# dusk-network/dusk-blindbidproof

Measured on AMD Instinct MI355X. Metric: blind-bid proofs/sec, higher is better.
Workload: dtype u32

## Files before the change

### __graft_entry__.py

```python
import os
import shutil
import subprocess
import sys

ROOT = os.path.dirname(os.path.abspath(__file__))
PKG = os.path.join(ROOT, "dusk_blindbidproof_amd")
CSRC = os.path.join(PKG, "csrc")
LIB = os.path.join(PKG, "libbbp_hip.so")
ORACLE_SO = os.path.join(ROOT, "oracle", "_build", "libbbp_oracle.so")
HOSTCHECK_SO = os.path.join(ROOT, "tests", "_build", "libhostcheck.so")
DEVCHECK_SO = {"chain": os.path.join(ROOT, "tests", "_build", "libbbp_devcheck.so"),
               "nochain": os.path.join(ROOT, "tests", "_build", "libbbp_devcheck_nochain.so")}
DEVCHECK_DEFS = {"chain": [], "nochain": ["-DBBP_FE_NO_CHAIN"]}


def _newer(target, sources):
    if not os.path.exists(target):
        return True
    t = os.path.getmtime(target)
    return any(os.path.getmtime(s) > t for s in sources)


def _run(cmd):
    print("+", " ".join(cmd), flush=True)
# ... 138 lines not shown
        _run(["g++", "-O1", "-g", "-std=c++17", "-fsanitize=address,undefined", "-fno-sanitize-recover=all", "-o", WIRE_FUZZ_BIN, src])
    return WIRE_FUZZ_BIN


VERIFY_PLAN_SAN_BIN = os.path.join(ROOT, "tests", "_build", "verify_plan_san")


def build_verify_plan_san(force=False):
    src = os.path.join(ROOT, "tests", "verify_plan_san.cpp")
    if force or _newer(VERIFY_PLAN_SAN_BIN, [src, os.path.join(ROOT, "tests", "host_check.cpp")] + _csrc_files((".h", ".inc"))):
        os.makedirs(os.path.dirname(VERIFY_PLAN_SAN_BIN), exist_ok=True)
        _run(["g++", "-O1", "-g", "-std=c++17", "-fsanitize=address,undefined", "-fno-sanitize-recover=all", "-o", VERIFY_PLAN_SAN_BIN, src])
    return VERIFY_PLAN_SAN_BIN


COMBINER_TSAN_BIN = os.path.join(ROOT, "tests", "_build", "combiner_tsan")


def build_combiner_tsan(force=False):
    srcs = [os.path.join(ROOT, "tests", "combiner_tsan.cpp"), os.path.join(CSRC, "submit.cpp")]
    if force or _newer(COMBINER_TSAN_BIN, srcs + [os.path.join(CSRC, "submit.h")]):
        os.makedirs(os.path.dirname(COMBINER_TSAN_BIN), exist_ok=True)
        _run(["g++", "-O1", "-g", "-std=c++17", "-fsanitize=thread", "-pthread", "-o", COMBINER_TSAN_BIN] + srcs)
    return COMBINER_TSAN_BIN


COMBINER_RULES_BIN = os.path.join(ROOT, "tests", "_build", "combiner_rules")


def build_combiner_rules(force=False):
# ... 56 lines not shown
```

### dusk_blindbidproof_amd/csrc/context.h

```cpp
#pragma once
#include <hip/hip_runtime.h>
#include <stdint.h>
#include <stdio.h>
#include <stdlib.h>
#include <string.h>

#include <atomic>
#include <condition_variable>
#include <map>
#include <mutex>
#include <new>
#include <stdexcept>
#include <string>
#include <vector>

#include "../../include/bbp.h"
#include "point.h"
#include "msm_plan.h"
#include "prove_io.h"
#include "prove_plan.h"
#include "scalar.h"
#include "verify_plan.h"
#include "verify_rows.h"

namespace bbp {

constexpr int MSM_POS = 256;
#ifndef BBP_MSM_T
#define BBP_MSM_T 128
#endif
constexpr int MSM_T = BBP_MSM_T;
#ifndef BBP_ACC_T
#define BBP_ACC_T 256
#endif
constexpr int ACC_T = BBP_ACC_T;
static_assert(ACC_T % MSM_T == 0, "the fold kernel deals the accumulate kernel's chunks to its lanes");
constexpr int MSM_G = MSM_K / MSM_T;
constexpr int MSM_LOG_G = MSM_T == 128 ? 3 : 4;
static_assert(MSM_T == 128 || MSM_T == 64, "the cross-lane fold is written for one or two wavefronts");
constexpr int FOLD_CLS = 2048 >> (FOLD_ROUND - 1);
constexpr int FOLD_NAF = 9;
constexpr int FOLD_W = 29;
constexpr int FOLD_M = 128;
constexpr int FOLD_K = FOLD_CLS * FOLD_M;
static_assert(SMALL_W == FOLD_W, "split MSMs recode at the generator-fold pass's width");
constexpr int PAD_BASES = 202;
constexpr unsigned PAD_BASE0 = BBP_NUM_BASES;
constexpr unsigned MRG_BASE0 = PAD_BASE0 + PAD_BASES;
constexpr int MRG_BASES = 2 * 2048;
constexpr unsigned MSM_SKIP_BASE = 0xffffffffu;
constexpr unsigned TAB_BASES = BBP_NUM_BASES + PAD_BASES + MRG_BASES;
constexpr int GE_WORDS = sizeof(ge) / 4;

struct DevBuf {
    void* p = nullptr;
    size_t cap = 0;
};

}

// ... 10 lines not shown
    hipStream_t copy = nullptr;
    hipStream_t side2 = nullptr;
    bbp::ProveKnobs knobs;
    bbp::ProveRuleState prove_state;
    bbp::VerifyKnobs vknobs;
    std::vector<hipStream_t> spare_streams;
    static constexpr int CALL_RING = 8;
    hipEvent_t ev_call[CALL_RING] = {};
    bool ev_call_valid[CALL_RING] = {};
    int last_prove_par = -1;
    static constexpr int MAX_SLICES = bbp::PROVE_MAX_SLICES;
    hipStream_t lane[MAX_SLICES] = {nullptr, nullptr, nullptr, nullptr};
    hipEvent_t ev_join[MAX_SLICES] = {nullptr, nullptr, nullptr, nullptr}, ev_stagger[MAX_SLICES] = {nullptr, nullptr, nullptr, nullptr};
    bbp::MsmKnobs msm_knobs;
    bool sort_lds_attr = false;
    bool sort_lds_attr1 = false;
    int debug_corrupt = 0;
    std::map<const void*, int> serial_attr;
    static constexpr int PROVE_BUFS = bbp::PROVE_BUFS;
    hipEvent_t ev_open[PROVE_BUFS] = {}, ev_done[PROVE_BUFS] = {};
    hipEvent_t ev_entry[PROVE_BUFS] = {};
    bool ev_done_valid[PROVE_BUFS] = {}, ev_open_valid[PROVE_BUFS] = {};
    int verify_serial_acc = 0;
    static constexpr int VACC_RING = 4;
    hipEvent_t ev_vacc[VACC_RING] = {};
    uint32_t vacc_seq = 0;
    bool vacc_valid = false;
    uint32_t seq_at_last_verify = 0;
    hipEvent_t ev_prep = nullptr;
    bool ev_prep_valid = false;
    hipEvent_t ev_draw = nullptr;
// ... 245 lines not shown
int hw_queues_state();
int32_t pool_prove_batch(bbp_ctx* pool, uint32_t B, uint32_t N, const uint8_t* in, const uint8_t* entropy, uint8_t* out, int32_t* status);
int32_t pool_prove_round(bbp_ctx* pool, uint32_t N, const uint8_t* round, uint32_t B, const uint8_t* bids, const uint8_t* entropy, uint8_t* rows_out,
                         uint64_t* toggles_out, int32_t* status);
int32_t pool_verify(bbp_ctx* pool, const VerifyRows& rows, const uint8_t* in, int32_t* status, uint32_t group, uint32_t* n_fallback);
int32_t verify_host(bbp_ctx* ctx, const VerifyRows& rows, const uint8_t* in, int32_t* status, uint32_t group, uint32_t* n_fallback);
int32_t pool_msm_batch(bbp_ctx* pool, uint32_t B, uint32_t n_terms, const uint8_t* scalars, uint32_t layout, uint8_t* out32);
int32_t pool_reject(bbp_ctx* pool, const char* what);
void pool_workers_start(bbp_ctx* pool);
void pool_workers_stop(bbp_ctx* pool);
int pool_member_numa_node(const bbp_ctx* pool, uint32_t i);

int32_t msm_launch(bbp_ctx* ctx, uint32_t n_msm, uint32_t n_terms, const u32* scalars_dev, const u32* base_idx_dev,
                   ge* out_points_dev, hipStream_t stream, uint32_t n_idx_sets = 1, int scratch_slot = 0, const u32* msm_map_dev = nullptr,
                   const u32* n_active_dev = nullptr, bool chain_acc = false);
int32_t fold_generators_launch(bbp_ctx* ctx, uint32_t n_proofs, const sc* g_dev, const sc* h_dev, ge* out_dev, hipStream_t stream,
                               int scratch_slot);
int32_t encode_launch(bbp_ctx* ctx, uint32_t n, const ge* pts_dev, uint8_t* out32_dev, hipStream_t stream);
size_t msm_scratch_bytes(uint32_t n_msm, uint32_t n_terms);
int32_t tail_btab_build(bbp_ctx* ctx);
size_t tail_btab_bytes();

}
```

### dusk_blindbidproof_amd/csrc/msm.hip

```cpp
#include "context.h"

namespace bbp {

#ifndef BBP_FOLD_PRIO
#define BBP_FOLD_PRIO 2
#endif
#ifndef BBP_MSM_WAVES
#define BBP_MSM_WAVES 2
#endif
#ifndef BBP_MSM_WAVES_MAX
#define BBP_MSM_WAVES_MAX 2
#endif

#ifdef BBP_MSM_PROF
__device__ unsigned long long g_msm_prof[8];
#define MSM_PROF_BEGIN() unsigned long long prof_t = wall_clock64()
#define MSM_PROF_MARK(i)                                                    \
    if (tid == 0) {                                                         \
        unsigned long long now_ = wall_clock64();                           \
        atomicAdd(&g_msm_prof[i], now_ - prof_t);                           \
        prof_t = now_;                                                      \
    }
#else
#define MSM_PROF_BEGIN()
// ... 87 lines not shown

template <int MODE>
__global__ __launch_bounds__(SORT_T) void k_msm_sort(const u32* __restrict__ scal_a, const u32* __restrict__ aux, u32 n_total, u32 n_idx_sets,
                                                      u32 n_sub, u32 split, u32* __restrict__ sorted_all, u32* __restrict__ cursor_all,
                                                      const u32* __restrict__ msm_map, const u32* __restrict__ n_active, u32* __restrict__ ticket) {
    constexpr int K = msm_geom<MODE>::K, NAF = msm_geom<MODE>::NAF, W = msm_geom<MODE>::W, G = K >= SORT_T ? K / SORT_T : 1;
    __shared__ u32 cursor[K + 1];
    __shared__ u32 part[SORT_T];
    const int tid = threadIdx.x;
    if (ticket && blockIdx.x == 0 && tid == 0) *ticket = 0;
    if (n_active && blockIdx.x >= *n_active) return;
    const size_t work = blockIdx.x, msm = work / split;
    const u32 i0 = (u32)(work % split) * n_sub;
    const u32 n = i0 < n_total ? min(n_sub, n_total - i0) : 0u;
    __builtin_amdgcn_s_setprio(3);
    const u32* sbase;
    const u32* base_idx = nullptr;
    u32 base0 = 0;
    if (MODE != 1) {
        const size_t src = msm_map ? (size_t)msm_map[msm] : msm;
        sbase = scal_a + (src * (size_t)n_total + i0) * 8;
        base_idx = aux + (size_t)(msm % n_idx_sets) * n_total + i0;
    } else {
        const u32 side = (u32)msm & 1u;
        sbase = (side ? aux : scal_a) + ((msm >> 1) * (size_t)2048 + i0) * 8;
        base0 = (side ? BBP_BASE_H0 : BBP_BASE_G0) + i0;
    }
    u32* sorted = sorted_all + work * (size_t)n_sub * W;
    auto key = [&](u32 i, u32 mag) -> u32 { return (MODE != 1 ? 0u : ((i0 + i) & (FOLD_CLS - 1)) * FOLD_M) + ((mag + 1) >> 1); };

    for (int k = tid; k <= K; k += SORT_T) cursor[k] = 0;
    __syncthreads();
    for (u32 i = tid; i < n; i += SORT_T) {
        const uint4* sp = reinterpret_cast<const uint4*>(sbase + (size_t)i * 8);
        uint4 lo = sp[0], hi = sp[1];
        const u32 s[8] = {lo.x, lo.y, lo.z, lo.w, hi.x, hi.y, hi.z, hi.w};
        if (MODE != 1 && base_idx[i] == MSM_SKIP_BASE) continue;
        sc_for_each_naf_digit<NAF>(s, [&](u32, u32 mag, u32) { atomicAdd(&cursor[key(i, mag)], 1u); });
    }
    __syncthreads();
    {
        u32 local = 0;
        for (int r = 1; r <= G; r++)
            if (tid * G + r <= K) local += cursor[tid * G + r];
        const int lane = tid & 63, wave = tid >> 6;
        u32 incl = local;
#pragma unroll
        for (int d = 1; d < 64; d <<= 1) {
            const u32 up = (u32)__shfl_up((int)incl, d, 64);
            if (lane >= d) incl += up;
        }
        if (lane == 63) part[wave] = incl;
// ... 10 lines not shown
        }
        __syncthreads();
        u32 base = part[wave] + incl - local;
        for (int r = 1; r <= G; r++) {
            if (tid * G + r > K) break;
            const u32 c = cursor[tid * G + r];
            cursor[tid * G + r] = base;
            base += c;
        }
    }
    __syncthreads();
    for (u32 i = tid; i < n; i += SORT_T) {
        const uint4* sp = reinterpret_cast<const uint4*>(sbase + (size_t)i * 8);
        uint4 lo = sp[0], hi = sp[1];
        const u32 s[8] = {lo.x, lo.y, lo.z, lo.w, hi.x, hi.y, hi.z, hi.w};
        if (MODE != 1 && base_idx[i] == MSM_SKIP_BASE) continue;
        const u32 tb = (MODE != 1 ? base_idx[i] : base0 + i) * MSM_POS;
        sc_for_each_naf_digit<NAF>(s, [&](u32 pos, u32 mag, u32 neg) {
            u32 at = atomicAdd(&cursor[key(i, mag)], 1u);
            sorted[at] = (tb + pos) | (neg << 31);
        });
    }
    __syncthreads();
    u32* cur_out = cursor_all + work * (size_t)(K + 1);
    for (int k = tid; k <= K; k += SORT_T) cur_out[k] = k ? cursor[k] : 0u;
}

template <int MODE> struct sort_cap { static constexpr u32 V = BBP_SORT_CAP; };
template <> struct sort_cap<1> { static constexpr u32 V = 8192; };

template <int MODE>
__global__ __launch_bounds__(SORT_T) void k_msm_sort_staged(const u32* __restrict__ scal_a, const u32* __restrict__ aux, u32 n_total, u32 n_idx_sets,
                                                             u32 n_sub, u32 split, u32* __restrict__ sorted_all, u32* __restrict__ cursor_all,
                                                             const u32* __restrict__ msm_map, const u32* __restrict__ n_active, u32 CAP, u32* __restrict__ ticket) {
    constexpr int K = msm_geom<MODE>::K, NAF = msm_geom<MODE>::NAF, W = msm_geom<MODE>::W, G = K >= SORT_T ? K / SORT_T : 1;
    extern __shared__ u32 stage[];
    __shared__ u32 start[K + 2];
    __shared__ u32 fill[K + 1];
    __shared__ u32 part[SORT_T];
    const int tid = threadIdx.x;
    if (ticket && blockIdx.x == 0 && tid == 0) *ticket = 0;
    if (n_active && blockIdx.x >= *n_active) return;
    const size_t work = blockIdx.x, msm = work / split;
    const u32 i0 = (u32)(work % split) * n_sub;
    const u32 n = i0 < n_total ? min(n_sub, n_total - i0) : 0u;
    __builtin_amdgcn_s_setprio(3);
    const u32* sbase;
    const u32* base_idx = nullptr;
    u32 base0 = 0;
    if (MODE != 1) {
        const size_t src = msm_map ? (size_t)msm_map[msm] : msm;
        sbase = scal_a + (src * (size_t)n_total + i0) * 8;
        base_idx = aux + (size_t)(msm % n_idx_sets) * n_total + i0;
    } else {
        const u32 side = (u32)msm & 1u;
        sbase = (side ? aux : scal_a) + ((msm >> 1) * (size_t)2048 + i0) * 8;
        base0 = (side ? BBP_BASE_H0 : BBP_BASE_G0) + i0;
    }
    u32* sorted = sorted_all + work * (size_t)n_sub * W;
    auto key = [&](u32 i, u32 mag) -> u32 { return (MODE != 1 ? 0u : ((i0 + i) & (FOLD_CLS - 1)) * FOLD_M) + ((mag + 1) >> 1); };

    for (int k = tid; k <= K; k += SORT_T) fill[k] = 0;
    __syncthreads();
    for (u32 i = tid; i < n; i += SORT_T) {
        const uint4* sp = reinterpret_cast<const uint4*>(sbase + (size_t)i * 8);
        uint4 lo = sp[0], hi = sp[1];
        const u32 s[8] = {lo.x, lo.y, lo.z, lo.w, hi.x, hi.y, hi.z, hi.w};
        if (MODE != 1 && base_idx[i] == MSM_SKIP_BASE) continue;
        sc_for_each_naf_digit<NAF>(s, [&](u32, u32 mag, u32) { atomicAdd(&fill[key(i, mag)], 1u); });
    }
    __syncthreads();
    {
        u32 local = 0;
        for (int r = 1; r <= G; r++)
            if (tid * G + r <= K) local += fill[tid * G + r];
        const int lane = tid & 63, wave = tid >> 6;
        u32 incl = local;
#pragma unroll
        for (int d = 1; d < 64; d <<= 1) {
            const u32 up = (u32)__shfl_up((int)incl, d, 64);
            if (lane >= d) incl += up;
        }
        if (lane == 63) part[wave] = incl;
// ... 27 lines not shown
        const bool direct = start[kb + 1] - base > CAP;
        u32 ke = kb + 1;
        if (!direct) {
            u32 lo = kb + 1, hi = (u32)K + 1;
            while (lo < hi) {
                const u32 mid = (lo + hi + 1) >> 1;
                if (start[mid] - base <= CAP) lo = mid; else hi = mid - 1;
            }
            ke = lo;
        }
        if (start[ke] != base) {
            for (u32 i = tid; i < n; i += SORT_T) {
                const uint4* sp = reinterpret_cast<const uint4*>(sbase + (size_t)i * 8);
                uint4 lo4 = sp[0], hi4 = sp[1];
                const u32 s[8] = {lo4.x, lo4.y, lo4.z, lo4.w, hi4.x, hi4.y, hi4.z, hi4.w};
                if (MODE != 1 && base_idx[i] == MSM_SKIP_BASE) continue;
                const u32 tb = (MODE != 1 ? base_idx[i] : base0 + i) * MSM_POS;
                sc_for_each_naf_digit<NAF>(s, [&](u32 pos, u32 mag, u32 neg) {
                    const u32 k = key(i, mag);
                    if (k >= kb && k < ke) {
                        const u32 at = start[k] + atomicAdd(&fill[k], 1u);
                        const u32 ent = (tb + pos) | (neg << 31);
                        if (direct) sorted[at] = ent; else stage[at - base] = ent;
                    }
                });
            }
            __syncthreads();
            if (!direct) {
                const u32 cnt = start[ke] - base;
                for (u32 i = tid; i < cnt; i += SORT_T) sorted[base + i] = stage[i];
            }
            __syncthreads();
        }
        kb = ke;
    }
    u32* cur_out = cursor_all + work * (size_t)(K + 1);
    for (int k = tid; k <= K; k += SORT_T) cur_out[k] = k ? start[k + 1] : 0u;
}

#ifndef BBP_ACC_WG
#define BBP_ACC_WG 256
#endif
constexpr int ACC_WG = BBP_ACC_WG, ACC_WGS = ACC_T / ACC_WG;
static_assert(ACC_T % ACC_WG == 0 && ACC_WG % 64 == 0, "accumulate workgroup geometry");

template <int MODE>
__global__ __launch_bounds__(ACC_WG) __attribute__((amdgpu_waves_per_eu(BBP_MSM_WAVES, BBP_MSM_WAVES_MAX)))
void k_msm_acc(const niels_row* __restrict__ ptable, const u32* __restrict__ sorted_all, const u32* __restrict__ cursor_all, u32 n ,
               ge* __restrict__ bsum_all, ge* __restrict__ psum_all, ge* __restrict__ out, const u32* __restrict__ n_active, u32* __restrict__ fault,
               u32 n_work, u32* __restrict__ ticket) {
    constexpr int K = msm_geom<MODE>::K, W = msm_geom<MODE>::W, G = K / MSM_T;
    __shared__ u32 cursor[K + 1];
// ... 113 lines not shown
        *dest = acc;
    }
#endif
#ifdef BBP_MSM_PROF
    if (tid == 0) atomicAdd(&g_msm_prof[6], clock64() - clk0);
#endif
    MSM_PROF_MARK(2);
    __threadfence_block();
    __syncthreads();
    MSM_PROF_MARK(3);
#ifdef BBP_ACC_PERSIST
  }
#endif
}

template <int MODE>
__global__ __launch_bounds__(MSM_T) void k_msm_fold(const u32* __restrict__ cursor_all, ge* __restrict__ bsum_all, const ge* __restrict__ psum_all,
                                                     ge* __restrict__ out, const u32* __restrict__ n_active) {
    constexpr int K = msm_geom<MODE>::K, G = K / MSM_T;
    __shared__ u32 cursor[K + 1];
    __shared__ u32 xch[GE_WORDS];
    const int tid = threadIdx.x;
    if (n_active && blockIdx.x >= *n_active) return;
    __builtin_amdgcn_s_setprio(BBP_FOLD_PRIO);
    const size_t msm = blockIdx.x;
    {
        const u32* cur_in = cursor_all + msm * (size_t)(K + 1);
        for (int k = tid; k <= K; k += MSM_T) cursor[k] = cur_in[k];
    }
    __syncthreads();
    const u32 E = cursor[K];
    ge* bsum = bsum_all + msm * (size_t)K;
    const ge* psum = psum_all + msm * (size_t)ACC_T;
#ifdef BBP_KO_FOLD
    if (MODE != 1) { if (tid == 0) out[msm] = bsum[0]; }
    else if (tid < FOLD_CLS) out[msm * FOLD_CLS + tid] = bsum[tid];
    return;
#endif
    for (u32 ch = tid; ch < (u32)ACC_T; ch += MSM_T) {
        const u32 c0 = (u32)(((u64)ch * E) / ACC_T), c1 = (u32)(((u64)(ch + 1) * E) / ACC_T);
        if (c0 >= c1) continue;
        u32 lo = 1, hi = K;
        while (lo < hi) {
            u32 mid = (lo + hi) >> 1;
            if (cursor[mid] > c0) hi = mid; else lo = mid + 1;
        }
        const u32 k_first = lo;
        const bool inside = cursor[lo - 1] < c0;
        const bool last_of_run = inside && !(c1 < E && c1 > cursor[k_first - 1] && c1 < cursor[k_first]);
        if (last_of_run) {
            ge part = psum[ch];
            for (int u = (int)ch - 1; u >= 0; u--) {
                const u32 cu = (u32)(((u64)u * E) / ACC_T), cu1 = (u32)(((u64)(u + 1) * E) / ACC_T);
                if (cu <= cursor[k_first - 1]) break;
                if (cu1 > cu) ge_add_nc(part, part, psum[u]);
            }
            ge head = bsum[k_first - 1];
            ge_add_nc(head, head, part);
            bsum[k_first - 1] = head;
        }
    }
    __threadfence_block();
    __syncthreads();

    ge running = ge_identity(), total = ge_identity();
    if constexpr (G == 1) {
        if (cursor[tid + 1] != cursor[tid]) running = bsum[tid];
        total = running;
    } else {
#pragma unroll 1
        for (int r = G; r >= 1; r--) {
            const u32 k = tid * G + r;
            if (cursor[k] != cursor[k - 1]) running = ge_add(running, bsum[k - 1]);
            total = ge_add(total, running);
        }
    }

    if constexpr (MODE != 1) {
        const int lane = tid & 63, wave = tid >> 6;
#pragma unroll 1
        for (int d = 1; d < 64; d <<= 1) {
            ge other = ge_shfl_down(running, d);
            if (lane + d < 64) running = ge_add(running, other);
        }
        if (MSM_T > 64) {
            if (tid == 64) xch_put(xch, running);
            __syncthreads();
            if (wave == 0) {
// ... 228 lines not shown
#pragma unroll 1
    for (int d = REDUCE_L / 2; d >= 1; d >>= 1) {
        const ge other = ge_shfl_down(acc, d);
        if ((int)j < d) acc = ge_add(acc, other);
    }
    if (o < n_out && j == 0) out[o] = acc;
}


struct MsmScratch {
    u32 *sorted, *cursor;
    ge *bsum, *psum, *tmp;
    u32* ticket;
    size_t bytes;
};
static MsmScratch msm_scratch_layout(void* base, size_t n_msm, size_t n_terms, size_t W, size_t K, size_t out_items = 1) {
    auto up = [](size_t x) { return (x + 255) / 256 * 256; };
    MsmScratch m;
    size_t o = 0;
    m.sorted = reinterpret_cast<u32*>(static_cast<u8*>(base) + o);
    o += up(n_msm * n_terms * W * sizeof(u32));
    m.cursor = reinterpret_cast<u32*>(static_cast<u8*>(base) + o);
    o += up(n_msm * (K + 1) * sizeof(u32));
    m.bsum = reinterpret_cast<ge*>(static_cast<u8*>(base) + o);
    o += n_msm * K * sizeof(ge);
    m.psum = reinterpret_cast<ge*>(static_cast<u8*>(base) + o);
    o += n_msm * ACC_T * sizeof(ge);
    m.tmp = reinterpret_cast<ge*>(static_cast<u8*>(base) + o);
    o += up(n_msm * out_items * sizeof(ge));
    m.ticket = reinterpret_cast<u32*>(static_cast<u8*>(base) + o);
    o += 256;
    m.bytes = o;
    return m;
}
size_t msm_scratch_bytes(uint32_t n_msm, uint32_t n_terms) {
    const u32 split = msm_split(n_msm, n_terms), n_sub = (n_terms + split - 1) / split;
    size_t a = msm_scratch_layout(nullptr, (size_t)n_msm * split, n_sub, MSM_W, MSM_K).bytes;
    if (split > 1) a = std::max(a, msm_scratch_layout(nullptr, (size_t)n_msm * split, n_sub, SMALL_W, SMALL_K).bytes);
    const size_t b = msm_scratch_layout(nullptr, n_msm, n_terms, MSM_W, MSM_K).bytes;
    return a > b ? a : b;
}

static inline u32 acc_grid(bbp_ctx*, u32 n_work) {
#ifdef BBP_ACC_PERSIST
    static const u32 cap = [] { const char* e = getenv("BBP_ACC_PERSIST_GRID"); return e ? (u32)atoi(e) : 512u; }();
    return n_work < cap ? n_work : cap;
#else
    return n_work * ACC_WGS;
#endif
}

int32_t fold_generators_launch(bbp_ctx* ctx, uint32_t n_proofs, const sc* g_dev, const sc* h_dev, ge* out_dev, hipStream_t stream,
                               int scratch_slot) {
    if (n_proofs == 0) return BBP_OK;
    const size_t n_msm = 2 * (size_t)n_proofs;
    const u32 split = msm_split((u32)n_msm, 2048), n_sub = (2048 + split - 1) / split;
    const size_t n_work = n_msm * split;
    DevBuf& scratch = ctx->slice_fold[scratch_slot];
    int32_t rc = dev_reserve(ctx, scratch, msm_scratch_layout(nullptr, n_work, n_sub, FOLD_W, FOLD_K, FOLD_CLS).bytes);
    if (rc) return rc;
    const MsmScratch m = msm_scratch_layout(scratch.p, n_work, n_sub, FOLD_W, FOLD_K, FOLD_CLS);
    {
        ScopedEvent ev(ctx, TAG_MSM_SORT, stream);
        if (ctx->msm_knobs.sort_staged & 2) {
            if (!ctx->sort_lds_attr1) {
                BBP_HIP_TRY(ctx, hipFuncSetAttribute((const void*)k_msm_sort_staged<1>, hipFuncAttributeMaxDynamicSharedMemorySize, (int)(sort_cap<1>::V * 4)));
                ctx->sort_lds_attr1 = true;
            }
            hipLaunchKernelGGL(k_msm_sort_staged<1>, dim3((u32)n_work), dim3(SORT_T), sort_cap<1>::V * 4, stream, (const u32*)g_dev, (const u32*)h_dev, 2048u, 1u,
                               n_sub, split, m.sorted, m.cursor, (const u32*)nullptr, (const u32*)nullptr, sort_cap<1>::V, m.ticket);
        } else
            hipLaunchKernelGGL(k_msm_sort<1>, dim3((u32)n_work), dim3(SORT_T), 0, stream, (const u32*)g_dev, (const u32*)h_dev, 2048u, 1u, n_sub, split,
                               m.sorted, m.cursor, (const u32*)nullptr, (const u32*)nullptr, m.ticket);
        BBP_HIP_TRY(ctx, hipGetLastError());
    }
    {
        ScopedEvent ev(ctx, TAG_MSM, stream);
        hipLaunchKernelGGL(k_msm_acc<1>, dim3(acc_grid(ctx, (u32)n_work)), dim3(ACC_WG), 0, stream, ctx->ptable, m.sorted, m.cursor, n_sub, m.bsum, m.psum,
                           split > 1 ? m.tmp : out_dev, (const u32*)nullptr, ctx->health, (u32)n_work, m.ticket);
        BBP_HIP_TRY(ctx, hipGetLastError());
    }
    ScopedEvent evf(ctx, TAG_MSM_FOLD, stream);
    hipLaunchKernelGGL(k_msm_fold<1>, dim3((u32)n_work), dim3(MSM_T), 0, stream, m.cursor, m.bsum, m.psum, split > 1 ? m.tmp : out_dev,
                       (const u32*)nullptr);
    BBP_HIP_TRY(ctx, hipGetLastError());
    if (split > 1) {
        const u32 n_out = (u32)n_msm * FOLD_CLS;
        hipLaunchKernelGGL(k_msm_reduce, dim3((n_out * REDUCE_L + 63) / 64), dim3(64), lds_token(ctx), stream, n_out, split, (u32)FOLD_CLS, m.tmp, out_dev);
        BBP_HIP_TRY(ctx, hipGetLastError());
    }
    return BBP_OK;
}

__global__ __launch_bounds__(64) void k_encode(const ge* __restrict__ pts, u32 n, u32* __restrict__ out_words) {
    u32 i = blockIdx.x * blockDim.x + threadIdx.x;
    if (i >= n) return;
    ge p = pts[i];
    u32 w[8];
    ge_encode_words(w, p);
    uint4* o = reinterpret_cast<uint4*>(out_words + (size_t)i * 8);
    o[0] = make_uint4(w[0], w[1], w[2], w[3]);
    o[1] = make_uint4(w[4], w[5], w[6], w[7]);
}
// ... 120 lines not shown
```

### dusk_blindbidproof_amd/csrc/msm_plan.h

```cpp
#pragma once
#include <stdint.h>
#include <stdlib.h>
#include <string.h>

#include <initializer_list>

namespace bbp {

constexpr int MSM_NAF = 12;
constexpr int MSM_W = 22;
constexpr int MSM_K = 1 << (MSM_NAF - 2);
constexpr int SMALL_NAF = 9;
constexpr int SMALL_K = 1 << (SMALL_NAF - 2);
constexpr int SMALL_W = 29;

#ifndef BBP_SORT_CAP
#define BBP_SORT_CAP 21504
#endif
constexpr uint32_t SORT_CAP_WIDE = 32768;
constexpr uint32_t SORT_WIDE_FROM = 3000;
constexpr uint32_t MSM_SPLIT_MAX = 16;

struct MsmKnobs {
    int sort_staged = 3;
// ... 64 lines not shown
    p.reduce = p.split > 1;
    if (p.split > 1 && k.msm_small) {
        p.geom = MsmPlan::SMALL;
        p.fold = MsmPlan::SMALL_FOLD;
        return p;
    }
    const bool wide = p.n_sub > SORT_WIDE_FROM;
    if ((k.sort_staged & 1) && (!wide || (k.sort_staged & 4))) {
        p.sort = wide ? MsmPlan::STAGED_WIDE : MsmPlan::STAGED;
        p.sort_cap = wide ? SORT_CAP_WIDE : (uint32_t)BBP_SORT_CAP;
    }
    p.fold = p.n_work >= (uint32_t)k.fold_half_from ? MsmPlan::HALF : MsmPlan::LANES128;
    return p;
}

}
```

### dusk_blindbidproof_amd/csrc/prover.hip

```cpp
#define BBP_KECCAK_WAVE 1
#include <string.h>

#include <functional>

#include "batch.h"
#include "hosthash.h"
#include "keccak_wave.h"
#include "scalarmul.h"
#include "witness.h"

namespace bbp {

#define BBP_THIN_PRIO() __builtin_amdgcn_s_setprio(3)
#ifndef BBP_LANE_KERNEL
#define BBP_LANE_KERNEL __launch_bounds__(64)
#endif


__device__ __forceinline__ void sc_to_bytes32(uint8_t* o, const sc& s) { sc_tobytes(o, s); }
__device__ __forceinline__ void words_to_bytes32(uint8_t* o, const u32* w) {
#pragma unroll
    for (int i = 0; i < 8; i++) {
        o[4 * i] = (uint8_t)w[i];
        o[4 * i + 1] = (uint8_t)(w[i] >> 8);
// ... 858 lines not shown
    for (int k = 0; k < TAIL_PIECES; k++) {
        ge cur = P;
        T[8 * k] = P;
#pragma unroll 1
        for (int i = 1; i < 8; i++) {
            cur = ge_add(cur, P);
            T[8 * k + i] = cur;
        }
        if (k < TAIL_PIECES - 1) {
#pragma unroll 1
            for (int i = 0; i < TAIL_PIECE_BITS; i++) P = ge_dbl(P);
        }
    }
}

__global__ void k_tail_init(u32 B, sc* __restrict__ g_all, sc* __restrict__ h_all) {
    BBP_THIN_PRIO();
    u32 t = blockIdx.x * blockDim.x + threadIdx.x;
    if (t >= B * FOLD_CLS) return;
    const u32 p = t / FOLD_CLS, k = t % FOLD_CLS;
    st_sc(&g_all[(size_t)p * 2048 + k], sc_one());
    st_sc(&h_all[(size_t)p * 2048 + k], sc_one());
}

#ifndef BBP_TAIL_SPLIT
#define BBP_TAIL_SPLIT 1
#endif
#ifndef BBP_TAIL_MERGE
#define BBP_TAIL_MERGE 1
#endif
#ifndef BBP_TAIL_BLK
#define BBP_TAIL_BLK (BBP_TAIL_SPLIT == 1 ? 256 : 320)
#endif
constexpr int TAIL_SPLIT = BBP_TAIL_SPLIT, TAIL_MERGE = BBP_TAIL_MERGE, TAIL_LS = TAIL_MERGE == 2 ? 17 : 33 * TAIL_SPLIT, TAIL_BLK = BBP_TAIL_BLK, TAIL_LP = 2 * TAIL_LS, TAIL_PPB = TAIL_BLK / TAIL_LP;
static_assert(TAIL_PIECES % TAIL_SPLIT == 0 && TAIL_PPB >= 1 && (TAIL_MERGE == 1 || (TAIL_MERGE == 2 && TAIL_SPLIT == 1)), "tail kernel geometry");
__global__ __launch_bounds__(TAIL_BLK) void k_tail_lr(u32 B, u32 n, u32 prev_round, u32 m, const u32* __restrict__ enc, merlin_transcript* __restrict__ tr,
                                                       const sc* __restrict__ misc, sc* __restrict__ a_all, sc* __restrict__ b_all,
// ... 485 lines not shown
    for (u32 r = 1; r <= 11 && r < tail_from; r++) {
        if (r > 1) LAUNCH(ctx, TAG_TRANSCRIPT, k_ipa_challenge, tgrid, 64, s, B, r - 1, m, bd.enc, bd.tr, bd.misc, tw);
        if (hp.wide_ipa)
            LAUNCH(ctx, TAG_IPA_SCALARS, k_ipa_round<IPA_BLK_WIDE>, B, IPA_BLK_WIDE, s, r, n1, bd.misc, bd.a, bd.b, bd.g, bd.h, bd.lr);
        else
            LAUNCH(ctx, TAG_IPA_SCALARS, k_ipa_round<IPA_BLK>, B, IPA_BLK, s, r, n1, bd.misc, bd.a, bd.b, bd.g, bd.h, bd.lr);
        if ((rc = msm_launch(ctx, 2 * B, 2049, (const u32*)bd.lr, c.idx_ipa + (size_t)(r - 1) * 2 * 2049, bd.lrpts, s, 2, slot))) return rc;
        LAUNCH(ctx, TAG_ENCODE, k_encode_strided, cdiv(2 * B, 64), 64, s, 2 * B, 2u, bd.lrpts, 2u, bd.enc, encw, 8 * (m + 8 + 2 * (r - 1)), 1u);
    }
    if (tail_from <= 11) {
        DevBuf& vt = ctx->slice_vtab[slot];
        if ((rc = dev_reserve(ctx, vt, (size_t)B * 2 * FOLD_CLS * TAIL_TAB * sizeof(ge)))) return rc;
        ge* ftab = static_cast<ge*>(vt.p);
        LAUNCH(ctx, TAG_TRANSCRIPT, k_ipa_challenge, tgrid, 64, s, B, tail_from - 1, m, bd.enc, bd.tr, bd.misc, tw);
        LAUNCH(ctx, TAG_IPA_SCALARS, k_ipa_round<IPA_BLK>, B, IPA_BLK, s, tail_from, n1, bd.misc, bd.a, bd.b, bd.g, bd.h, (sc*)nullptr);
        if ((rc = fold_generators_launch(ctx, B, bd.g, bd.h, bd.fpts, s, slot))) return rc;
        LAUNCH(ctx, TAG_VARBASE, k_tail_init, cdiv(B * FOLD_CLS, 64), 64, s, B, bd.g, bd.h);
        LAUNCH(ctx, TAG_VARBASE, k_tail_tables, cdiv(B * 2 * FOLD_CLS, 64), 64, s, B * 2 * FOLD_CLS, bd.fpts, ftab);
        for (u32 r = tail_from; r <= 11; r++) {
            const u32 n = 1024u >> (r - 1);
            LAUNCH(ctx, TAG_VARBASE, k_tail_lr, cdiv(B, TAIL_PPB), TAIL_BLK, s, B, n, r > tail_from ? r - 1 : 0u, m, bd.enc, bd.tr, bd.misc, bd.a, bd.b, bd.g, bd.h, ftab,
                   ctx->btab, bd.lrpts);
            LAUNCH(ctx, TAG_ENCODE, k_encode_strided, cdiv(2 * B, 64), 64, s, 2 * B, 2u, bd.lrpts, 2u, bd.enc, encw, 8 * (m + 8 + 2 * (r - 1)), 1u);
        }
    }
    LAUNCH(ctx, TAG_TRANSCRIPT, k_ipa_final, tgrid, 64, s, B, m, bd.enc, bd.tr, bd.misc, bd.a, bd.b, tw);
    if (out_guard) BBP_HIP_TRY(ctx, hipStreamWaitEvent(s, out_guard, 0));
    LAUNCH(ctx, TAG_TRANSCRIPT, k_assemble, cdiv(B, 64), 64, s, B, m, bd.enc, bd.misc, out_dev);
    return BBP_OK;
}

int32_t debug_read_misc(bbp_ctx* ctx, u32 B, u32 N, u32 proof, uint8_t* out) {
// ... 13 lines not shown
```

Baseline: 22650.

## Replace generator-fold MSM with dedicated class-strided fold sort and accumulate kernels

Swaps the generic MODE-1 MSM sort/accumulate path for folding generators with new k_fold_sort and k_fold_acc kernels. The sort bins one scalar per class stride into 128 buckets, and each accumulate lane handles one class, so the per-class bucket key expansion goes away. The fold now takes n1 and the u challenge so it can handle the partially-active boundary generator. k_tail_init seeds h with yipow instead of one, which shifts the y-inverse factor out of the folded scalars. A new FoldPlan computes the scratch layout. Correctness depends on the tag and class masking logic being exact.

```diff
diff --git a/__graft_entry__.py b/__graft_entry__.py
--- a/__graft_entry__.py
+++ b/__graft_entry__.py
@@ -176,6 +176,17 @@
     return VERIFY_PLAN_SAN_BIN
 
 
+FOLD_PLAN_SAN_BIN = os.path.join(ROOT, "tests", "_build", "fold_plan_san")
+
+
+def build_fold_plan_san(force=False):
+    src = os.path.join(ROOT, "tests", "fold_plan_san.cpp")
+    if force or _newer(FOLD_PLAN_SAN_BIN, [src, os.path.join(CSRC, "msm_plan.h")]):
+        os.makedirs(os.path.dirname(FOLD_PLAN_SAN_BIN), exist_ok=True)
+        _run(["g++", "-O1", "-g", "-std=c++17", "-fsanitize=address,undefined", "-fno-sanitize-recover=all", "-o", FOLD_PLAN_SAN_BIN, src])
+    return FOLD_PLAN_SAN_BIN
+
+
 COMBINER_TSAN_BIN = os.path.join(ROOT, "tests", "_build", "combiner_tsan")
 
 
diff --git a/dusk_blindbidproof_amd/csrc/context.h b/dusk_blindbidproof_amd/csrc/context.h
--- a/dusk_blindbidproof_amd/csrc/context.h
+++ b/dusk_blindbidproof_amd/csrc/context.h
@@ -38,12 +38,7 @@
 constexpr int MSM_G = MSM_K / MSM_T;
 constexpr int MSM_LOG_G = MSM_T == 128 ? 3 : 4;
 static_assert(MSM_T == 128 || MSM_T == 64, "the cross-lane fold is written for one or two wavefronts");
-constexpr int FOLD_CLS = 2048 >> (FOLD_ROUND - 1);
-constexpr int FOLD_NAF = 9;
-constexpr int FOLD_W = 29;
-constexpr int FOLD_M = 128;
-constexpr int FOLD_K = FOLD_CLS * FOLD_M;
-static_assert(SMALL_W == FOLD_W, "split MSMs recode at the generator-fold pass's width");
+static_assert(FOLD_CLS == 2048 >> (FOLD_ROUND - 1), "one class per folded generator of the first tail round");
 constexpr int PAD_BASES = 202;
 constexpr unsigned PAD_BASE0 = BBP_NUM_BASES;
 constexpr unsigned MRG_BASE0 = PAD_BASE0 + PAD_BASES;
@@ -84,7 +79,6 @@
     hipEvent_t ev_join[MAX_SLICES] = {nullptr, nullptr, nullptr, nullptr}, ev_stagger[MAX_SLICES] = {nullptr, nullptr, nullptr, nullptr};
     bbp::MsmKnobs msm_knobs;
     bool sort_lds_attr = false;
-    bool sort_lds_attr1 = false;
     int debug_corrupt = 0;
     std::map<const void*, int> serial_attr;
     static constexpr int PROVE_BUFS = bbp::PROVE_BUFS;
@@ -360,8 +354,8 @@
 int32_t msm_launch(bbp_ctx* ctx, uint32_t n_msm, uint32_t n_terms, const u32* scalars_dev, const u32* base_idx_dev,
                    ge* out_points_dev, hipStream_t stream, uint32_t n_idx_sets = 1, int scratch_slot = 0, const u32* msm_map_dev = nullptr,
                    const u32* n_active_dev = nullptr, bool chain_acc = false);
-int32_t fold_generators_launch(bbp_ctx* ctx, uint32_t n_proofs, const sc* g_dev, const sc* h_dev, ge* out_dev, hipStream_t stream,
-                               int scratch_slot);
+int32_t fold_generators_launch(bbp_ctx* ctx, uint32_t n_proofs, const sc* g_dev, const sc* h_dev, uint32_t n1, const sc* u_dev, uint32_t u_stride,
+                               ge* out_dev, hipStream_t stream, int scratch_slot);
 int32_t encode_launch(bbp_ctx* ctx, uint32_t n, const ge* pts_dev, uint8_t* out32_dev, hipStream_t stream);
 size_t msm_scratch_bytes(uint32_t n_msm, uint32_t n_terms);
 int32_t tail_btab_build(bbp_ctx* ctx);
diff --git a/dusk_blindbidproof_amd/csrc/msm.hip b/dusk_blindbidproof_amd/csrc/msm.hip
--- a/dusk_blindbidproof_amd/csrc/msm.hip
+++ b/dusk_blindbidproof_amd/csrc/msm.hip
@@ -125,20 +125,11 @@
     const u32 i0 = (u32)(work % split) * n_sub;
     const u32 n = i0 < n_total ? min(n_sub, n_total - i0) : 0u;
     __builtin_amdgcn_s_setprio(3);
-    const u32* sbase;
-    const u32* base_idx = nullptr;
-    u32 base0 = 0;
-    if (MODE != 1) {
-        const size_t src = msm_map ? (size_t)msm_map[msm] : msm;
-        sbase = scal_a + (src * (size_t)n_total + i0) * 8;
-        base_idx = aux + (size_t)(msm % n_idx_sets) * n_total + i0;
-    } else {
-        const u32 side = (u32)msm & 1u;
-        sbase = (side ? aux : scal_a) + ((msm >> 1) * (size_t)2048 + i0) * 8;
-        base0 = (side ? BBP_BASE_H0 : BBP_BASE_G0) + i0;
-    }
+    const size_t src = msm_map ? (size_t)msm_map[msm] : msm;
+    const u32* sbase = scal_a + (src * (size_t)n_total + i0) * 8;
+    const u32* base_idx = aux + (size_t)(msm % n_idx_sets) * n_total + i0;
     u32* sorted = sorted_all + work * (size_t)n_sub * W;
-    auto key = [&](u32 i, u32 mag) -> u32 { return (MODE != 1 ? 0u : ((i0 + i) & (FOLD_CLS - 1)) * FOLD_M) + ((mag + 1) >> 1); };
+    auto key = [&](u32, u32 mag) -> u32 { return (mag + 1) >> 1; };
 
     for (int k = tid; k <= K; k += SORT_T) cursor[k] = 0;
     __syncthreads();
@@ -146,7 +137,7 @@
         const uint4* sp = reinterpret_cast<const uint4*>(sbase + (size_t)i * 8);
         uint4 lo = sp[0], hi = sp[1];
         const u32 s[8] = {lo.x, lo.y, lo.z, lo.w, hi.x, hi.y, hi.z, hi.w};
-        if (MODE != 1 && base_idx[i] == MSM_SKIP_BASE) continue;
+        if (base_idx[i] == MSM_SKIP_BASE) continue;
         sc_for_each_naf_digit<NAF>(s, [&](u32, u32 mag, u32) { atomicAdd(&cursor[key(i, mag)], 1u); });
     }
     __syncthreads();
@@ -187,8 +178,8 @@
         const uint4* sp = reinterpret_cast<const uint4*>(sbase + (size_t)i * 8);
         uint4 lo = sp[0], hi = sp[1];
         const u32 s[8] = {lo.x, lo.y, lo.z, lo.w, hi.x, hi.y, hi.z, hi.w};
-        if (MODE != 1 && base_idx[i] == MSM_SKIP_BASE) continue;
-        const u32 tb = (MODE != 1 ? base_idx[i] : base0 + i) * MSM_POS;
+        if (base_idx[i] == MSM_SKIP_BASE) continue;
+        const u32 tb = base_idx[i] * MSM_POS;
         sc_for_each_naf_digit<NAF>(s, [&](u32 pos, u32 mag, u32 neg) {
             u32 at = atomicAdd(&cursor[key(i, mag)], 1u);
             sorted[at] = (tb + pos) | (neg << 31);
@@ -198,9 +189,6 @@
     u32* cur_out = cursor_all + work * (size_t)(K + 1);
     for (int k = tid; k <= K; k += SORT_T) cur_out[k] = k ? cursor[k] : 0u;
 }
-
-template <int MODE> struct sort_cap { static constexpr u32 V = BBP_SORT_CAP; };
-template <> struct sort_cap<1> { static constexpr u32 V = 8192; };
 
 template <int MODE>
 __global__ __launch_bounds__(SORT_T) void k_msm_sort_staged(const u32* __restrict__ scal_a, const u32* __restrict__ aux, u32 n_total, u32 n_idx_sets,
@@ -218,20 +206,11 @@
     const u32 i0 = (u32)(work % split) * n_sub;
     const u32 n = i0 < n_total ? min(n_sub, n_total - i0) : 0u;
     __builtin_amdgcn_s_setprio(3);
-    const u32* sbase;
-    const u32* base_idx = nullptr;
-    u32 base0 = 0;
-    if (MODE != 1) {
-        const size_t src = msm_map ? (size_t)msm_map[msm] : msm;
-        sbase = scal_a + (src * (size_t)n_total + i0) * 8;
-        base_idx = aux + (size_t)(msm % n_idx_sets) * n_total + i0;
-    } else {
-        const u32 side = (u32)msm & 1u;
-        sbase = (side ? aux : scal_a) + ((msm >> 1) * (size_t)2048 + i0) * 8;
-        base0 = (side ? BBP_BASE_H0 : BBP_BASE_G0) + i0;
-    }
+    const size_t src = msm_map ? (size_t)msm_map[msm] : msm;
+    const u32* sbase = scal_a + (src * (size_t)n_total + i0) * 8;
+    const u32* base_idx = aux + (size_t)(msm % n_idx_sets) * n_total + i0;
     u32* sorted = sorted_all + work * (size_t)n_sub * W;
-    auto key = [&](u32 i, u32 mag) -> u32 { return (MODE != 1 ? 0u : ((i0 + i) & (FOLD_CLS - 1)) * FOLD_M) + ((mag + 1) >> 1); };
+    auto key = [&](u32, u32 mag) -> u32 { return (mag + 1) >> 1; };
 
     for (int k = tid; k <= K; k += SORT_T) fill[k] = 0;
     __syncthreads();
@@ -239,7 +218,7 @@
         const uint4* sp = reinterpret_cast<const uint4*>(sbase + (size_t)i * 8);
         uint4 lo = sp[0], hi = sp[1];
         const u32 s[8] = {lo.x, lo.y, lo.z, lo.w, hi.x, hi.y, hi.z, hi.w};
-        if (MODE != 1 && base_idx[i] == MSM_SKIP_BASE) continue;
+        if (base_idx[i] == MSM_SKIP_BASE) continue;
         sc_for_each_naf_digit<NAF>(s, [&](u32, u32 mag, u32) { atomicAdd(&fill[key(i, mag)], 1u); });
     }
     __syncthreads();
@@ -297,8 +276,8 @@
                 const uint4* sp = reinterpret_cast<const uint4*>(sbase + (size_t)i * 8);
                 uint4 lo4 = sp[0], hi4 = sp[1];
                 const u32 s[8] = {lo4.x, lo4.y, lo4.z, lo4.w, hi4.x, hi4.y, hi4.z, hi4.w};
-                if (MODE != 1 && base_idx[i] == MSM_SKIP_BASE) continue;
-                const u32 tb = (MODE != 1 ? base_idx[i] : base0 + i) * MSM_POS;
+                if (base_idx[i] == MSM_SKIP_BASE) continue;
+                const u32 tb = base_idx[i] * MSM_POS;
                 sc_for_each_naf_digit<NAF>(s, [&](u32 pos, u32 mag, u32 neg) {
                     const u32 k = key(i, mag);
                     if (k >= kb && k < ke) {
@@ -319,6 +298,81 @@
     }
     u32* cur_out = cursor_all + work * (size_t)(K + 1);
     for (int k = tid; k <= K; k += SORT_T) cur_out[k] = k ? start[k + 1] : 0u;
+}
+
+constexpr u32 FOLD_ENT_ROW = 0x00ffffffu;
+constexpr int FOLD_SORT_T = 128, FOLD_SLOTS_MAX = (int)FOLD_T + 1;
+static_assert(FOLD_SORT_T >= FOLD_M && FOLD_SORT_T >= FOLD_SLOTS_MAX && FOLD_SORT_T == 128, "one lane per bucket and per scalar, two wavefronts");
+static_assert((u64)(TAB_BASES + FOLD_CLS) * MSM_POS <= FOLD_ENT_ROW, "a row index fits its field");
+
+__global__ __launch_bounds__(FOLD_SORT_T) void k_fold_sort(const sc* __restrict__ g_all, const sc* __restrict__ h_all, u32 n1, const sc* __restrict__ u_all,
+                                                            u32 u_stride, u32 t_sub, u32 split, u32 stride ,
+                                                            u32* __restrict__ sorted_all, u32* __restrict__ cursor_all) {
+    constexpr int K = FOLD_M;
+    __shared__ u32 start[K + 2];
+    __shared__ u32 fill[K + 1];
+    __shared__ u32 part[2];
+    __shared__ u32 stage[FOLD_SLOTS_MAX * FOLD_W];
+    const u32 tid = threadIdx.x;
+    __builtin_amdgcn_s_setprio(3);
+    const size_t work = blockIdx.x, pass = work / split, p = pass >> 1;
+    const u32 side = (u32)pass & 1u;
+    const u32 t0 = (u32)(work % split) * t_sub;
+    const u32 nt = t0 < FOLD_T ? min(t_sub, FOLD_T - t0) : 0u;
+    const u32 tb = n1 / FOLD_CLS, c = n1 % FOLD_CLS;
+    const bool divided = c != 0 && tb >= t0 && tb < t0 + nt;
+    const bool extra = divided && tid == nt, live = tid < nt || extra;
+    const u32 t = extra ? tb : t0 + tid;
+    u32 s[8] = {0, 0, 0, 0, 0, 0, 0, 0};
+    u32 tag = 1u << 30;
+    if (live) {
+        const uint4* sp = reinterpret_cast<const uint4*>((side ? h_all : g_all) + p * 2048 + (size_t)t * FOLD_CLS);
+        const uint4 lo = sp[0], hi = sp[1];
+        sc x = sc{{lo.x, lo.y, lo.z, lo.w, hi.x, hi.y, hi.z, hi.w}};
+        if (extra) {
+            const uint4* up = reinterpret_cast<const uint4*>(u_all + p * u_stride);
+            const uint4 ul = up[0], uh = up[1];
+            x = sc_mul(x, sc{{ul.x, ul.y, ul.z, ul.w, uh.x, uh.y, uh.z, uh.w}});
+        }
+#pragma unroll
+        for (int w = 0; w < 8; w++) s[w] = x.v[w];
+        if (divided && t == tb) tag = (c << 24) | (extra ? 1u << 30 : 0u);
+    }
+    const u32 row0 = ((side ? BBP_BASE_H0 : BBP_BASE_G0) + t * FOLD_CLS) * MSM_POS;
+
+    for (u32 k = tid; k <= (u32)K; k += FOLD_SORT_T) fill[k] = 0;
+    __syncthreads();
+    if (live) sc_for_each_naf_digit<FOLD_NAF>(s, [&](u32, u32 mag, u32) { atomicAdd(&fill[(mag + 1) >> 1], 1u); });
+    __syncthreads();
+    {
+        const u32 lane = tid & 63, wave = tid >> 6;
+        const u32 local = fill[tid + 1];
+        u32 incl = local;
+#pragma unroll
+        for (int d = 1; d < 64; d <<= 1) {
+            const u32 up = (u32)__shfl_up((int)incl, d, 64);
+            if (lane >= (u32)d) incl += up;
+        }
+        if (lane == 63) part[wave] = incl;
+        __syncthreads();
+        const u32 base = (wave ? part[0] : 0u) + incl - local;
+        start[tid + 1] = base;
+        fill[tid + 1] = 0;
+        if (tid == (u32)K - 1) start[K + 1] = base + local;
+        if (tid == 0) start[0] = 0;
+    }
+    __syncthreads();
+    if (live)
+        sc_for_each_naf_digit<FOLD_NAF>(s, [&](u32 pos, u32 mag, u32 neg) {
+            const u32 k = (mag + 1) >> 1;
+            stage[start[k] + atomicAdd(&fill[k], 1u)] = (row0 + pos) | tag | (neg << 31);
+        });
+    __syncthreads();
+    u32* sorted = sorted_all + work * (size_t)stride;
+    const u32 E = min(start[K + 1], stride);
+    for (u32 i = tid; i < E; i += FOLD_SORT_T) sorted[i] = stage[i];
+    u32* cur_out = cursor_all + work * (size_t)(K + 1);
+    for (u32 k = tid; k <= (u32)K; k += FOLD_SORT_T) cur_out[k] = k ? start[k + 1] : 0u;
 }
 
 #ifndef BBP_ACC_WG
@@ -462,22 +516,83 @@
 #endif
 }
 
+constexpr int FOLD_CHUNKS = ACC_T / FOLD_CLS;
+static_assert(ACC_T % FOLD_CLS == 0 && ACC_WG == ACC_T && FOLD_CLS == 32, "one accumulate workgroup per pass, half a wavefront per chunk");
+
+__global__ __launch_bounds__(ACC_WG) __attribute__((amdgpu_waves_per_eu(BBP_MSM_WAVES, BBP_MSM_WAVES_MAX)))
+void k_fold_acc(const niels_row* __restrict__ ptable, const u32* __restrict__ sorted_all, const u32* __restrict__ cursor_all, u32 stride ,
+                ge* __restrict__ bsum_all, ge* __restrict__ psum_all, u32* __restrict__ fault) {
+    constexpr int K = FOLD_M;
+    __shared__ u32 cursor[K + 1];
+    const size_t work = blockIdx.x;
+    const u32 tid = threadIdx.x, cls = tid % FOLD_CLS, ch = tid / FOLD_CLS;
+    const u32* sorted = sorted_all + work * (size_t)stride;
+    {
+        const u32* cur_in = cursor_all + work * (size_t)(K + 1);
+        for (u32 k = tid; k <= (u32)K; k += ACC_WG) cursor[k] = min(cur_in[k], stride);
+    }
+    __syncthreads();
+    const u32 E = cursor[K];
+    ge* bsum = bsum_all + work * (size_t)FOLD_K + (size_t)cls * FOLD_M;
+    ge* psum = psum_all + work * (size_t)ACC_T;
+    const u32 c0 = (u32)(((u64)ch * E) / FOLD_CHUNKS), c1 = (u32)(((u64)(ch + 1) * E) / FOLD_CHUNKS);
+    if (c0 >= c1) return;
+    u32 lo = 1, hi = K;
+    while (lo < hi) {
+        const u32 mid = (lo + hi) >> 1;
+        if (cursor[mid] > c0) hi = mid; else lo = mid + 1;
+    }
+    u32 k = lo, kend = cursor[k];
+    ge* dest = cursor[k - 1] < c0 ? &psum[tid] : &bsum[k - 1];
+    ge acc = ge_identity();
+    auto row_of = [&](u32 entry) -> row_regs {
+        u32 row = (entry & FOLD_ENT_ROW) + cls * MSM_POS;
+        if (row > (u32)(TAB_BASES * MSM_POS - 1)) {
+            row = (u32)(TAB_BASES * MSM_POS - 1);
+            atomicOr(fault, 1u);
+        }
+        return load_row_at(ptable + row, entry >> 31);
+    };
+    u32 ent_cur = sorted[c0];
+    u32 ent_nxt = (c0 + 1 < c1) ? sorted[c0 + 1] : 0u;
+    row_regs row = row_of(ent_cur);
+    for (u32 e = c0; e < c1; e++) {
+        if (e == kend) {
+            *dest = acc;
+            acc = ge_identity();
+            do { k++; kend = cursor[k]; } while (kend == e);
+            dest = &bsum[k - 1];
+        }
+        const row_regs cur = row;
+        const bool neg = ent_cur >> 31;
+        const bool mine = (cls >= ((ent_cur >> 24) & 63u)) == (bool)((ent_cur >> 30) & 1u);
+        ent_cur = ent_nxt;
+        if (e + 1 < c1) row = row_of(ent_cur);
+        if (e + 2 < c1) ent_nxt = sorted[e + 2];
+        if (mine) acc = ge_madd_row(acc, cur, neg);
+    }
+    *dest = acc;
+}
+
 template <int MODE>
 __global__ __launch_bounds__(MSM_T) void k_msm_fold(const u32* __restrict__ cursor_all, ge* __restrict__ bsum_all, const ge* __restrict__ psum_all,
                                                      ge* __restrict__ out, const u32* __restrict__ n_active) {
     constexpr int K = msm_geom<MODE>::K, G = K / MSM_T;
-    __shared__ u32 cursor[K + 1];
+    constexpr int KC = MODE == 1 ? FOLD_M : K;
+    constexpr u32 PST = MODE == 1 ? (u32)FOLD_CLS : 1u;
+    constexpr u32 NCH = (u32)ACC_T / PST;
+    __shared__ u32 cursor[KC + 1];
     __shared__ u32 xch[GE_WORDS];
     const int tid = threadIdx.x;
     if (n_active && blockIdx.x >= *n_active) return;
     __builtin_amdgcn_s_setprio(BBP_FOLD_PRIO);
     const size_t msm = blockIdx.x;
     {
-        const u32* cur_in = cursor_all + msm * (size_t)(K + 1);
-        for (int k = tid; k <= K; k += MSM_T) cursor[k] = cur_in[k];
-    }
-    __syncthreads();
-    const u32 E = cursor[K];
+        const u32* cur_in = cursor_all + msm * (size_t)(KC + 1);
+        for (int k = tid; k <= KC; k += MSM_T) cursor[k] = cur_in[k];
+    }
+    __syncthreads();
+    const u32 E = cursor[KC];
     ge* bsum = bsum_all + msm * (size_t)K;
     const ge* psum = psum_all + msm * (size_t)ACC_T;
 #ifdef BBP_KO_FOLD
@@ -485,10 +600,12 @@
     else if (tid < FOLD_CLS) out[msm * FOLD_CLS + tid] = bsum[tid];
     return;
 #endif
-    for (u32 ch = tid; ch < (u32)ACC_T; ch += MSM_T) {
-        const u32 c0 = (u32)(((u64)ch * E) / ACC_T), c1 = (u32)(((u64)(ch + 1) * E) / ACC_T);
+    for (u32 w = tid; w < (u32)ACC_T; w += MSM_T) {
+        const u32 ch = w / PST, cls = w % PST;
+        ge* bsum_c = bsum + (size_t)cls * KC;
+        const u32 c0 = (u32)(((u64)ch * E) / NCH), c1 = (u32)(((u64)(ch + 1) * E) / NCH);
         if (c0 >= c1) continue;
-        u32 lo = 1, hi = K;
+        u32 lo = 1, hi = KC;
         while (lo < hi) {
             u32 mid = (lo + hi) >> 1;
             if (cursor[mid] > c0) hi = mid; else lo = mid + 1;
@@ -497,15 +614,15 @@
         const bool inside = cursor[lo - 1] < c0;
         const bool last_of_run = inside && !(c1 < E && c1 > cursor[k_first - 1] && c1 < cursor[k_first]);
         if (last_of_run) {
-            ge part = psum[ch];
+            ge part = psum[w];
             for (int u = (int)ch - 1; u >= 0; u--) {
-                const u32 cu = (u32)(((u64)u * E) / ACC_T), cu1 = (u32)(((u64)(u + 1) * E) / ACC_T);
+                const u32 cu = (u32)(((u64)u * E) / NCH), cu1 = (u32)(((u64)(u + 1) * E) / NCH);
                 if (cu <= cursor[k_first - 1]) break;
-                if (cu1 > cu) ge_add_nc(part, part, psum[u]);
-            }
-            ge head = bsum[k_first - 1];
+                if (cu1 > cu) ge_add_nc(part, part, psum[(u32)u * PST + cls]);
+            }
+            ge head = bsum_c[k_first - 1];
             ge_add_nc(head, head, part);
-            bsum[k_first - 1] = head;
+            bsum_c[k_first - 1] = head;
         }
     }
     __threadfence_block();
@@ -518,8 +635,8 @@
     } else {
 #pragma unroll 1
         for (int r = G; r >= 1; r--) {
-            const u32 k = tid * G + r;
-            if (cursor[k] != cursor[k - 1]) running = ge_add(running, bsum[k - 1]);
+            const u32 k = tid * G + r, kc = MODE == 1 ? k - (k - 1) / KC * KC : k;
+            if (cursor[kc] != cursor[kc - 1]) running = ge_add(running, bsum[k - 1]);
             total = ge_add(total, running);
         }
     }
@@ -778,7 +895,7 @@
     u32* ticket;
     size_t bytes;
 };
-static MsmScratch msm_scratch_layout(void* base, size_t n_msm, size_t n_terms, size_t W, size_t K, size_t out_items = 1) {
+static MsmScratch msm_scratch_layout(void* base, size_t n_msm, size_t n_terms, size_t W, size_t K) {
     auto up = [](size_t x) { return (x + 255) / 256 * 256; };
     MsmScratch m;
     size_t o = 0;
@@ -791,7 +908,7 @@
     m.psum = reinterpret_cast<ge*>(static_cast<u8*>(base) + o);
     o += n_msm * ACC_T * sizeof(ge);
     m.tmp = reinterpret_cast<ge*>(static_cast<u8*>(base) + o);
-    o += up(n_msm * out_items * sizeof(ge));
+    o += up(n_msm * sizeof(ge));
     m.ticket = reinterpret_cast<u32*>(static_cast<u8*>(base) + o);
     o += 256;
     m.bytes = o;
@@ -814,43 +931,33 @@
 #endif
 }
 
-int32_t fold_generators_launch(bbp_ctx* ctx, uint32_t n_proofs, const sc* g_dev, const sc* h_dev, ge* out_dev, hipStream_t stream,
-                               int scratch_slot) {
+int32_t fold_generators_launch(bbp_ctx* ctx, uint32_t n_proofs, const sc* g_dev, const sc* h_dev, uint32_t n1, const sc* u_dev, uint32_t u_stride,
+                               ge* out_dev, hipStream_t stream, int scratch_slot) {
     if (n_proofs == 0) return BBP_OK;
-    const size_t n_msm = 2 * (size_t)n_proofs;
-    const u32 split = msm_split((u32)n_msm, 2048), n_sub = (2048 + split - 1) / split;
-    const size_t n_work = n_msm * split;
+    const FoldPlan fp = plan_fold(ctx->msm_knobs, n_proofs, sizeof(ge), ACC_T);
     DevBuf& scratch = ctx->slice_fold[scratch_slot];
-    int32_t rc = dev_reserve(ctx, scratch, msm_scratch_layout(nullptr, n_work, n_sub, FOLD_W, FOLD_K, FOLD_CLS).bytes);
+    int32_t rc = dev_reserve(ctx, scratch, fp.bytes);
     if (rc) return rc;
-    const MsmScratch m = msm_scratch_layout(scratch.p, n_work, n_sub, FOLD_W, FOLD_K, FOLD_CLS);
+    u8* base = static_cast<u8*>(scratch.p);
+    u32 *sorted = reinterpret_cast<u32*>(base + fp.o_sorted), *cursor = reinterpret_cast<u32*>(base + fp.o_cursor);
+    ge *bsum = reinterpret_cast<ge*>(base + fp.o_bsum), *psum = reinterpret_cast<ge*>(base + fp.o_psum), *tmp = reinterpret_cast<ge*>(base + fp.o_tmp);
+    ge* folded = fp.split > 1 ? tmp : out_dev;
     {
         ScopedEvent ev(ctx, TAG_MSM_SORT, stream);
-        if (ctx->msm_knobs.sort_staged & 2) {
-            if (!ctx->sort_lds_attr1) {
-                BBP_HIP_TRY(ctx, hipFuncSetAttribute((const void*)k_msm_sort_staged<1>, hipFuncAttributeMaxDynamicSharedMemorySize, (int)(sort_cap<1>::V * 4)));
-                ctx->sort_lds_attr1 = true;
-            }
-            hipLaunchKernelGGL(k_msm_sort_staged<1>, dim3((u32)n_work), dim3(SORT_T), sort_cap<1>::V * 4, stream, (const u32*)g_dev, (const u32*)h_dev, 2048u, 1u,
-                               n_sub, split, m.sorted, m.cursor, (const u32*)nullptr, (const u32*)nullptr, sort_cap<1>::V, m.ticket);
-        } else
-            hipLaunchKernelGGL(k_msm_sort<1>, dim3((u32)n_work), dim3(SORT_T), 0, stream, (const u32*)g_dev, (const u32*)h_dev, 2048u, 1u, n_sub, split,
-                               m.sorted, m.cursor, (const u32*)nullptr, (const u32*)nullptr, m.ticket);
+        hipLaunchKernelGGL(k_fold_sort, dim3(fp.n_work), dim3(FOLD_SORT_T), 0, stream, g_dev, h_dev, n1, u_dev, u_stride, fp.t_sub, fp.split, fp.entries, sorted, cursor);
         BBP_HIP_TRY(ctx, hipGetLastError());
     }
     {
         ScopedEvent ev(ctx, TAG_MSM, stream);
-        hipLaunchKernelGGL(k_msm_acc<1>, dim3(acc_grid(ctx, (u32)n_work)), dim3(ACC_WG), 0, stream, ctx->ptable, m.sorted, m.cursor, n_sub, m.bsum, m.psum,
-                           split > 1 ? m.tmp : out_dev, (const u32*)nullptr, ctx->health, (u32)n_work, m.ticket);
+        hipLaunchKernelGGL(k_fold_acc, dim3(fp.n_work), dim3(ACC_WG), 0, stream, ctx->ptable, sorted, cursor, fp.entries, bsum, psum, ctx->health);
         BBP_HIP_TRY(ctx, hipGetLastError());
     }
     ScopedEvent evf(ctx, TAG_MSM_FOLD, stream);
-    hipLaunchKernelGGL(k_msm_fold<1>, dim3((u32)n_work), dim3(MSM_T), 0, stream, m.cursor, m.bsum, m.psum, split > 1 ? m.tmp : out_dev,
-                       (const u32*)nullptr);
+    hipLaunchKernelGGL(k_msm_fold<1>, dim3(fp.n_work), dim3(MSM_T), 0, stream, cursor, bsum, psum, folded, (const u32*)nullptr);
     BBP_HIP_TRY(ctx, hipGetLastError());
-    if (split > 1) {
-        const u32 n_out = (u32)n_msm * FOLD_CLS;
-        hipLaunchKernelGGL(k_msm_reduce, dim3((n_out * REDUCE_L + 63) / 64), dim3(64), lds_token(ctx), stream, n_out, split, (u32)FOLD_CLS, m.tmp, out_dev);
+    if (fp.split > 1) {
+        const u32 n_out = 2 * n_proofs * FOLD_CLS;
+        hipLaunchKernelGGL(k_msm_reduce, dim3((n_out * REDUCE_L + 63) / 64), dim3(64), lds_token(ctx), stream, n_out, fp.split, (u32)FOLD_CLS, tmp, out_dev);
         BBP_HIP_TRY(ctx, hipGetLastError());
     }
     return BBP_OK;
diff --git a/dusk_blindbidproof_amd/csrc/msm_plan.h b/dusk_blindbidproof_amd/csrc/msm_plan.h
--- a/dusk_blindbidproof_amd/csrc/msm_plan.h
+++ b/dusk_blindbidproof_amd/csrc/msm_plan.h
@@ -102,4 +102,40 @@
     return p;
 }
 
+constexpr int FOLD_CLS = 32;
+constexpr int FOLD_NAF = 9;
+constexpr int FOLD_W = 29;
+constexpr int FOLD_M = 128;
+constexpr int FOLD_K = FOLD_CLS * FOLD_M;
+constexpr uint32_t FOLD_T = 2048 / FOLD_CLS;
+static_assert(SMALL_W == FOLD_W, "split MSMs recode at the generator-fold pass's width");
+
+struct FoldPlan {
+    uint32_t split = 1;
+    uint32_t t_sub = FOLD_T;
+    uint32_t n_work = 0;
+    uint32_t slots = 0;
+    uint32_t entries = 0;
+    size_t o_sorted = 0, o_cursor = 0, o_bsum = 0, o_psum = 0, o_tmp = 0, bytes = 0;
+};
+
+inline FoldPlan plan_fold(const MsmKnobs& k, uint32_t n_proofs, size_t point_bytes, uint32_t acc_t) {
+    FoldPlan p;
+    const uint32_t want = msm_split(k, 2 * n_proofs, 2048);
+    p.t_sub = (FOLD_T + want - 1) / want;
+    p.split = (FOLD_T + p.t_sub - 1) / p.t_sub;
+    p.n_work = 2 * n_proofs * p.split;
+    p.slots = p.t_sub + 1;
+    p.entries = p.slots * FOLD_W;
+    auto up = [](size_t x) { return (x + 255) / 256 * 256; };
+    const size_t w = p.n_work;
+    p.o_sorted = 0;
+    p.o_cursor = p.o_sorted + up(w * p.entries * sizeof(uint32_t));
+    p.o_bsum = p.o_cursor + up(w * (FOLD_M + 1) * sizeof(uint32_t));
+    p.o_psum = p.o_bsum + up(w * FOLD_K * point_bytes);
+    p.o_tmp = p.o_psum + up(w * acc_t * point_bytes);
+    p.bytes = p.o_tmp + up(w * FOLD_CLS * point_bytes);
+    return p;
 }
+
+}
diff --git a/dusk_blindbidproof_amd/csrc/prover.hip b/dusk_blindbidproof_amd/csrc/prover.hip
--- a/dusk_blindbidproof_amd/csrc/prover.hip
+++ b/dusk_blindbidproof_amd/csrc/prover.hip
@@ -896,13 +896,13 @@
     }
 }
 
-__global__ void k_tail_init(u32 B, sc* __restrict__ g_all, sc* __restrict__ h_all) {
+__global__ void k_tail_init(u32 B, const sc* __restrict__ yipow, sc* __restrict__ g_all, sc* __restrict__ h_all) {
     BBP_THIN_PRIO();
     u32 t = blockIdx.x * blockDim.x + threadIdx.x;
     if (t >= B * FOLD_CLS) return;
     const u32 p = t / FOLD_CLS, k = t % FOLD_CLS;
     st_sc(&g_all[(size_t)p * 2048 + k], sc_one());
-    st_sc(&h_all[(size_t)p * 2048 + k], sc_one());
+    st_sc(&h_all[(size_t)p * 2048 + k], ld_sc(&yipow[(size_t)p * 2048 + k]));
 }
 
 #ifndef BBP_TAIL_SPLIT
@@ -1418,8 +1418,8 @@
         ge* ftab = static_cast<ge*>(vt.p);
         LAUNCH(ctx, TAG_TRANSCRIPT, k_ipa_challenge, tgrid, 64, s, B, tail_from - 1, m, bd.enc, bd.tr, bd.misc, tw);
         LAUNCH(ctx, TAG_IPA_SCALARS, k_ipa_round<IPA_BLK>, B, IPA_BLK, s, tail_from, n1, bd.misc, bd.a, bd.b, bd.g, bd.h, (sc*)nullptr);
-        if ((rc = fold_generators_launch(ctx, B, bd.g, bd.h, bd.fpts, s, slot))) return rc;
-        LAUNCH(ctx, TAG_VARBASE, k_tail_init, cdiv(B * FOLD_CLS, 64), 64, s, B, bd.g, bd.h);
+        if ((rc = fold_generators_launch(ctx, B, bd.g, bd.h, n1, bd.misc + MS_U, (u32)MS_COUNT, bd.fpts, s, slot))) return rc;
+        LAUNCH(ctx, TAG_VARBASE, k_tail_init, cdiv(B * FOLD_CLS, 64), 64, s, B, bd.yipow, bd.g, bd.h);
         LAUNCH(ctx, TAG_VARBASE, k_tail_tables, cdiv(B * 2 * FOLD_CLS, 64), 64, s, B * 2 * FOLD_CLS, bd.fpts, ftab);
         for (u32 r = tail_from; r <= 11; r++) {
             const u32 n = 1024u >> (r - 1);
```

Result: faster. 23390, median of 6 (+3.3%).
